# IN2-ViAUn/Exploration-of-Potential

Measured on AMD Instinct MI355X. Metric: training images/sec, YOLOX-l 24p 640x640 bf16, higher is better.
Workload: dtype bf16; 1 GPU; YOLOX-l-24p (CSPDarknet53+PAFPN+24p head) train step, 640x640, batch 20/GPU, 10 GTs/img, SimOTA + 24-circle GIoU loss, SGD nesterov; global_batch=20, parallelism=dp1, hip_graph=forward and backward as two lanes of captured segments, loss, update

## Files before the change

### exploration-of-potential_amd/csrc/elementwise.hip

```cpp
#include <stdio.h>
#include <stdlib.h>
#include "common.h"

namespace {

constexpr int MAX_BLOCKS = 2048;

__device__ __forceinline__ void load8(const bf16* p, float (&v)[8]) {
    bf16x8 t = *reinterpret_cast<const bf16x8*>(p);
#pragma unroll
    for (int i = 0; i < 8; ++i) v[i] = (float)t[i];
}
__device__ __forceinline__ void store8(bf16* p, const float (&v)[8]) {
    bf16x8 t;
#pragma unroll
    for (int i = 0; i < 8; ++i) t[i] = (bf16)v[i];
    *reinterpret_cast<bf16x8*>(p) = t;
}

struct RowMap {
    int tpr, rpb;
    __device__ RowMap(int C, int nt = 256) { tpr = C >> 3; rpb = tpr >= nt ? 1 : nt / tpr; }
};

template <int ACT, bool RES>
__global__ __launch_bounds__(256) void bn_act_fwd_kernel(const bf16* z, long ld_z, const long long* stats, int reps,
                                                         const float* gamma, const float* beta, float* rmean,
                                                         float* rvar, long* nbt, long* nbt2, float* save, bf16* y, long ld_y,
                                                         const bf16* res_, long ld_res, long M, int C, float eps,
                                                         float momentum) {
    constexpr int act = ACT;
    const bf16* res = RES ? res_ : nullptr;
    extern __shared__ float lds[];
    const int CP = C + (C >> 3);
    float* sc = lds;
    float* sh = lds + CP;
    auto pad = [](int c) { return c + (c >> 3); };
    for (int c = threadIdx.x; c < C; c += 256) {
        long long i1 = 0, i2 = 0;
        const float gmm = gamma[c], bta = beta[c];
        for (int rb = 0; rb < reps; rb += 8) {
            long long a[8], b[8];
#pragma unroll
            for (int r = 0; r < 8; ++r) {
                const int rr = rb + r < reps ? rb + r : rb;
                a[r] = stats[(long)rr * 2 * C + c];
                b[r] = stats[(long)rr * 2 * C + C + c];
            }
#pragma unroll
            for (int r = 0; r < 8; ++r) {
                i1 += rb + r < reps ? a[r] : 0ll;
                i2 += rb + r < reps ? b[r] : 0ll;
            }
        }
        const float mean = from_fix(i1) / (float)M;
        float var = from_fix(i2) / (float)M - mean * mean;
        var = var < 0.f ? 0.f : var;
        const float invstd = rsqrtf(var + eps);
        const float s_ = gmm * invstd;
        sc[pad(c)] = s_;
        sh[pad(c)] = bta - mean * s_;
        if (blockIdx.x == 0) {
            save[c] = mean;
            save[C + c] = invstd;
            if (rmean) {
                const float unb = M > 1 ? var * (float)M / (float)(M - 1) : var;
                rmean[c] = (1.f - momentum) * rmean[c] + momentum * mean;
                rvar[c] = (1.f - momentum) * rvar[c] + momentum * unb;
            }
        }
    }
    if (blockIdx.x == 0 && threadIdx.x == 0) {
        if (nbt) *nbt += 1;
        if (nbt2) *nbt2 += 1;
    }
    __syncthreads();
    const int cgs = C >> 3;
    const long total = M * cgs;
    const long stride = (long)gridDim.x * 256;
    constexpr int U = 4;
    const bool fixed_group = stride % cgs == 0;
    const int g_fixed = (int)(((long)blockIdx.x * 256 + threadIdx.x) % cgs);
    float rsc[8], rsh[8];
#pragma unroll
    for (int j = 0; j < 8; ++j) { rsc[j] = sc[g_fixed * 9 + j]; rsh[j] = sh[g_fixed * 9 + j]; }
    const long m_fixed = ((long)blockIdx.x * 256 + threadIdx.x) / cgs, m_step = stride / cgs;
    int it = 0;
    for (long i = (long)blockIdx.x * 256 + threadIdx.x; i < total; i += U * stride, ++it) {
        long mm[U];
        int gg[U];
        bf16x8 v[U], r[U];
#pragma unroll
        for (int k = 0; k < U; ++k) {
            const long ik = i + k * stride;
            const bool ok = ik < total;
            if (fixed_group) {
                mm[k] = ok ? m_fixed + (long)(it * U + k) * m_step : -1;
                gg[k] = g_fixed;
            } else {
                mm[k] = ok ? ik / cgs : -1;
                gg[k] = ok ? (int)(ik - mm[k] * cgs) : 0;
            }
            if (ok) {
                v[k] = *reinterpret_cast<const bf16x8*>(z + mm[k] * ld_z + gg[k] * 8);
                if constexpr (RES) r[k] = *reinterpret_cast<const bf16x8*>(res + mm[k] * ld_res + gg[k] * 8);
            }
        }
#pragma unroll
        for (int k = 0; k < U; ++k) {
            if (mm[k] < 0) break;
            bf16x8 o;
#pragma unroll
            for (int j = 0; j < 8; ++j) {
                const float a_ = fixed_group ? rsc[j] : sc[gg[k] * 9 + j];
                const float b_ = fixed_group ? rsh[j] : sh[gg[k] * 9 + j];
                const float u = fmaf((float)v[k][j], a_, b_);
                if constexpr (RES) o[j] = (bf16)(act_fwd(u, act) + (float)r[k][j]);
                else o[j] = (bf16)act_fwd(u, act);
            }
            *reinterpret_cast<bf16x8*>(y + mm[k] * ld_y + gg[k] * 8) = o;
        }
    }
}


template <int UNROLL, int NT, int ACT>
__device__ __forceinline__ void bn_bwd_reduce_body(const bf16* dy, long ld_dy, const bf16* z, long ld_z,
                                                   const float* save, const float* gamma,
                                                   const float* beta, long long* dgamma, long long* dbeta,
                                                   long M, int C, int reps, const int bid, const int nblk) {
    constexpr int act = ACT;
    __shared__ float red[NT][8 + 1];
    const RowMap rm(C, NT);
    const int tid = threadIdx.x;
    for (int cg0 = 0; cg0 < (C >> 3); cg0 += NT) {
        const int cg = cg0 + tid % rm.tpr;
        const int slot = rm.tpr >= NT ? 0 : tid / rm.tpr;
        const bool active = slot < rm.rpb && cg < (C >> 3);
        float sg[8] = {0, 0, 0, 0, 0, 0, 0, 0}, sb[8] = {0, 0, 0, 0, 0, 0, 0, 0};
        if (active) {
            const long step = (long)nblk * rm.rpb;
            const long m_first = (long)bid * rm.rpb + slot;
            bf16x8 vdy[UNROLL], vz[UNROLL];
#pragma unroll
            for (int k = 0; k < UNROLL; ++k) {
                const long mm = m_first + k * step < M ? m_first + k * step : (m_first < M ? m_first : 0);
                vdy[k] = *reinterpret_cast<const bf16x8*>(dy + mm * ld_dy + cg * 8);
                vz[k] = *reinterpret_cast<const bf16x8*>(z + mm * ld_z + cg * 8);
            }
            __builtin_amdgcn_sched_barrier(0);
            float sc[8], sh[8], iv[8], mi[8];
#pragma unroll
            for (int j = 0; j < 8; ++j) {
                const int c = cg * 8 + j;
                const float mean = save[c], inv = save[C + c];
                sc[j] = gamma[c] * inv; sh[j] = beta[c] - mean * sc[j]; iv[j] = inv; mi[j] = mean * inv;
            }
            for (long m = m_first; m < M; m += UNROLL * step) {
#pragma unroll
                for (int k = 0; k < UNROLL; ++k) {
                    if (m + k * step >= M) break;
#pragma unroll
                    for (int j = 0; j < 8; ++j) {
                        const float zz = (float)vz[k][j];
                        const float du = (float)vdy[k][j] * act_grad(fmaf(zz, sc[j], sh[j]), act);
                        sb[j] += du;
                        sg[j] = fmaf(du, fmaf(zz, iv[j], -mi[j]), sg[j]);
                    }
                }
                if (m + UNROLL * step < M) {
#pragma unroll
                    for (int k = 0; k < UNROLL; ++k) {
                        const long mn = m + (UNROLL + k) * step;
                        const long mm = mn < M ? mn : m;
                        vdy[k] = *reinterpret_cast<const bf16x8*>(dy + mm * ld_dy + cg * 8);
                        vz[k] = *reinterpret_cast<const bf16x8*>(z + mm * ld_z + cg * 8);
                    }
                }
            }
        }
        const int ngrp = min(min(rm.tpr, NT), (C >> 3) - cg0);
#pragma unroll
        for (int half = 0; half < 2; ++half) {
#pragma unroll
            for (int j = 0; j < 8; ++j) red[tid][j] = half ? sb[j] : sg[j];
            __syncthreads();
            for (int t = tid; t < ngrp * 8; t += NT) {
                const int g = t >> 3, v = t & 7;
                float a = 0.f;
                for (int sl = 0; sl < rm.rpb; ++sl) a += red[sl * rm.tpr + g][v];
                long long* dst = (half ? dbeta : dgamma) + (long)(bid % reps) * 2 * C + (cg0 + g) * 8 + v;
                atomicAdd((unsigned long long*)dst, (unsigned long long)to_fix_g(a));
            }
            __syncthreads();
        }
    }
}

template <int UNROLL, int NT, int ACT>
__global__ __launch_bounds__(NT) void bn_act_bwd_reduce_kernel(const bf16* dy, long ld_dy, const bf16* z, long ld_z,
                                                               const float* save, const float* gamma,
                                                               const float* beta, long long* dgamma, long long* dbeta,
                                                               long M, int C, int reps) {
    bn_bwd_reduce_body<UNROLL, NT, ACT>(dy, ld_dy, z, ld_z, save, gamma, beta, dgamma, dbeta, M, C, reps, (int)blockIdx.x, (int)gridDim.x);
}

template <int UNROLL, int ACT, bool ACC, bool COH>
__device__ __forceinline__ void bn_bwd_apply_body(const bf16* dy, long ld_dy, const bf16* z, long ld_z,
                                                  const float* save, const float* gamma, const float* beta,
                                                  const long long* dgamma, const long long* dbeta, float* ggrad,
                                                  float* bgrad, bf16* dz, long ld_dz, long M, int C, int reps, const int bid, const int nblk) {
    constexpr int act = ACT;
    const RowMap rm(C);
    const int tid = threadIdx.x;
    const float invM = 1.f / (float)M;
    extern __shared__ float folded[];
    for (int i = tid; i < 2 * C; i += 256) {
        const long long* src = i < C ? dgamma + i : dbeta + (i - C);
        long long acc = 0;
        bool bad = false;
        for (int rb = 0; rb < reps; rb += 8) {
            long long a[8];
#pragma unroll
            for (int r = 0; r < 8; ++r) {
                const long long* q = src + (long)(rb + r < reps ? rb + r : rb) * 2 * C;
                a[r] = COH ? __hip_atomic_load(q, __ATOMIC_RELAXED, __HIP_MEMORY_SCOPE_AGENT) : *q;
            }
#pragma unroll
            for (int r = 0; r < 8; ++r) {
                acc += rb + r < reps ? a[r] : 0ll;
                bad = bad || fixg_bad(a[r]);
            }
        }
        folded[i] = bad ? __builtin_nanf("") : from_fix_g(acc);
    }
    __syncthreads();
    for (int cg = tid % rm.tpr; cg < (C >> 3); cg += 256) {
        const int slot = rm.tpr >= 256 ? 0 : tid / rm.tpr;
        if (slot >= rm.rpb) break;
        float sc[8], sh[8], k1[8], k2[8], k3[8];
        float cm[8], ci[8], cg_[8], cb[8], csg[8], csb[8];
        {
            const f32x4* pm = reinterpret_cast<const f32x4*>(save + cg * 8);
            const f32x4* pi = reinterpret_cast<const f32x4*>(save + C + cg * 8);
            const f32x4* pg = reinterpret_cast<const f32x4*>(gamma + cg * 8);
            const f32x4* pb = reinterpret_cast<const f32x4*>(beta + cg * 8);
            const f32x4 m0 = pm[0], m1 = pm[1], i0 = pi[0], i1 = pi[1], g0 = pg[0], g1 = pg[1], b0 = pb[0], b1 = pb[1];
            const f32x4 s0 = *reinterpret_cast<const f32x4*>(folded + cg * 8), s1 = *reinterpret_cast<const f32x4*>(folded + cg * 8 + 4);
            const f32x4 t0 = *reinterpret_cast<const f32x4*>(folded + C + cg * 8), t1 = *reinterpret_cast<const f32x4*>(folded + C + cg * 8 + 4);
#pragma unroll
            for (int j = 0; j < 4; ++j) {
                cm[j] = m0[j]; cm[4 + j] = m1[j]; ci[j] = i0[j]; ci[4 + j] = i1[j]; cg_[j] = g0[j]; cg_[4 + j] = g1[j]; cb[j] = b0[j]; cb[4 + j] = b1[j];
                csg[j] = s0[j]; csg[4 + j] = s1[j]; csb[j] = t0[j]; csb[4 + j] = t1[j];
            }
        }
#pragma unroll
        for (int j = 0; j < 8; ++j) {
            const float mean = cm[j], inv = ci[j], g = cg_[j];
            const float sg_ = csg[j], sb_ = csb[j];
            sc[j] = g * inv; sh[j] = cb[j] - mean * sc[j];
            k1[j] = g * inv;
            k3[j] = k1[j] * inv * (sg_ * invM);
            k2[j] = k1[j] * (sb_ * invM) - k3[j] * mean;
        }
        if (bid == 0 && slot == 0 && ggrad) {
            f32x4* pgg = reinterpret_cast<f32x4*>(ggrad + cg * 8);
            f32x4* pbg = reinterpret_cast<f32x4*>(bgrad + cg * 8);
            f32x4 a0 = pgg[0], a1 = pgg[1], c0 = pbg[0], c1 = pbg[1];
#pragma unroll
            for (int j = 0; j < 4; ++j) {
                a0[j] += csg[j]; a1[j] += csg[4 + j];
                c0[j] += csb[j]; c1[j] += csb[4 + j];
            }
            pgg[0] = a0; pgg[1] = a1; pbg[0] = c0; pbg[1] = c1;
        }
        const long step = (long)nblk * rm.rpb;
        for (long m = (long)bid * rm.rpb + slot; m < M; m += UNROLL * step) {
            bf16x8 vdy[UNROLL], vz[UNROLL];
#pragma unroll
            for (int k = 0; k < UNROLL; ++k) {
                const long mm = m + k * step;
                if (mm < M) {
                    vdy[k] = __builtin_nontemporal_load(reinterpret_cast<const bf16x8*>(dy + mm * ld_dy + cg * 8));
                    vz[k] = __builtin_nontemporal_load(reinterpret_cast<const bf16x8*>(z + mm * ld_z + cg * 8));
                }
            }
#pragma unroll
            for (int k = 0; k < UNROLL; ++k) {
                const long mm = m + k * step;
                if (mm >= M) break;
                bf16x8 o;
#pragma unroll
                for (int j = 0; j < 8; ++j) {
                    const float zz = (float)vz[k][j];
                    const float du = (float)vdy[k][j] * act_grad(fmaf(zz, sc[j], sh[j]), act);
                    o[j] = (bf16)fmaf(-k3[j], zz, fmaf(k1[j], du, -k2[j]));
                }
                if (ACC) {
                    const bf16x8 old = *reinterpret_cast<const bf16x8*>(dz + mm * ld_dz + cg * 8);
#pragma unroll
                    for (int j = 0; j < 8; ++j) o[j] = (bf16)((float)old[j] + (float)o[j]);
                }
                *reinterpret_cast<bf16x8*>(dz + mm * ld_dz + cg * 8) = o;
            }
        }
    }
}

template <int UNROLL, int ACT, bool ACC = false>
__global__ __launch_bounds__(256) void bn_act_bwd_apply_kernel(const bf16* dy, long ld_dy, const bf16* z, long ld_z,
                                                               const float* save, const float* gamma, const float* beta,
                                                               const long long* dgamma, const long long* dbeta, float* ggrad,
                                                               float* bgrad, bf16* dz, long ld_dz, long M, int C, int reps) {
    bn_bwd_apply_body<UNROLL, ACT, ACC, false>(dy, ld_dy, z, ld_z, save, gamma, beta, dgamma, dbeta, ggrad, bgrad, dz, ld_dz, M, C, reps,
                                               (int)blockIdx.x, (int)gridDim.x);
}

__device__ unsigned g_bn_barrier_timeouts;

template <int ACT>
__global__ __launch_bounds__(256) void bn_act_bwd_fused_kernel(const bf16* dy, long ld_dy, const bf16* z, long ld_z,
                                                               const float* save, const float* gamma, const float* beta,
                                                               long long* dgamma, long long* dbeta, float* ggrad, float* bgrad,
                                                               bf16* dz, long ld_dz, long M, int C, int reps, unsigned* bar) {
    const int bid = (int)blockIdx.x, nblk = (int)gridDim.x;
    bn_bwd_reduce_body<4, 256, ACT>(dy, ld_dy, z, ld_z, save, gamma, beta, dgamma, dbeta, M, C, reps, bid, nblk);
    __syncthreads();
    if (threadIdx.x == 0) {
        __threadfence();
        __hip_atomic_fetch_add(bar, 1u, __ATOMIC_RELEASE, __HIP_MEMORY_SCOPE_AGENT);
        int tries = 0;
        while (__hip_atomic_load(bar, __ATOMIC_ACQUIRE, __HIP_MEMORY_SCOPE_AGENT) < (unsigned)nblk) {
            __builtin_amdgcn_s_sleep(2);
            if (++tries > (1 << 16)) { atomicAdd(&g_bn_barrier_timeouts, 1u); break; }
        }
    }
    __syncthreads();
    bn_bwd_apply_body<4, ACT, false, true>(dy, ld_dy, z, ld_z, save, gamma, beta, dgamma, dbeta, ggrad, bgrad, dz, ld_dz, M, C, reps, bid, nblk);
}

int flat_grid(long M, int C, int per_thread) {
    long blocks = (M * (C >> 3) + 256L * per_thread - 1) / (256L * per_thread);
    return (int)(blocks < 1 ? 1 : (blocks > MAX_BLOCKS ? MAX_BLOCKS : blocks));
}
int rows_grid(long M, int C, int rows_per_thread, int max_blocks, int nt = 256) {
    int tpr = C >> 3;
    int rpb = tpr >= nt ? 1 : nt / tpr;
    long blocks = (M + (long)rpb * rows_per_thread - 1) / ((long)rpb * rows_per_thread);
    return (int)(blocks < 1 ? 1 : (blocks > max_blocks ? max_blocks : blocks));
}

__global__ __launch_bounds__(256) void stem_pack_kernel(const float* img, bf16* rows, int B, int IH, int IW, int ld) {
    constexpr int TP = 32;
    __shared__ __attribute__((aligned(16))) bf16 tile[TP][120];
    const int FH = IH >> 1, FW = IW >> 1;
    const long npix = (long)B * FH * FW;
    const int chunks = ld >> 3;
    for (long p0 = (long)blockIdx.x * TP; p0 < npix; p0 += (long)gridDim.x * TP) {
        for (int it = threadIdx.x; it < 9 * TP; it += 256) {
            const int tap = it / TP, lp = it - tap * TP;
            const long pix = p0 + lp;
            float v[12] = {0.f, 0.f, 0.f, 0.f, 0.f, 0.f, 0.f, 0.f, 0.f, 0.f, 0.f, 0.f};
            if (pix < npix) {
                const int n = (int)(pix / ((long)FH * FW));
                const int rem = (int)(pix - (long)n * FH * FW);
                const int oy = rem / FW, ox = rem - oy * FW;
                const int fy = oy + tap / 3 - 1, fx = ox + tap % 3 - 1;
                if (fy >= 0 && fy < FH && fx >= 0 && fx < FW) {
#pragma unroll
                    for (int ch = 0; ch < 3; ++ch)
#pragma unroll
                        for (int yp = 0; yp < 2; ++yp) {
                            const float2 t = *reinterpret_cast<const float2*>(img + (((long)n * 3 + ch) * IH + 2 * fy + yp) * IW + 2 * fx);
                            v[(0 * 2 + yp) * 3 + ch] = t.x;
                            v[(1 * 2 + yp) * 3 + ch] = t.y;
                        }
                }
            }
#pragma unroll
            for (int j = 0; j < 12; ++j) tile[lp][tap * 12 + j] = (bf16)v[j];
        }
        if (threadIdx.x < TP) {
#pragma unroll
            for (int j = 108; j < 120; ++j) tile[threadIdx.x][j] = (bf16)0.f;
        }
        __syncthreads();
        for (int it = threadIdx.x; it < TP * chunks; it += 256) {
            const int lp = it / chunks, c = it - lp * chunks;
            const long pix = p0 + lp;
            if (pix >= npix) continue;
            bf16x8 o = {0, 0, 0, 0, 0, 0, 0, 0};
            if (c * 8 < 120) o = *reinterpret_cast<const bf16x8*>(&tile[lp][c * 8]);
            *reinterpret_cast<bf16x8*>(rows + pix * ld + c * 8) = o;
        }
        __syncthreads();
    }
}

__global__ __launch_bounds__(256) void focus_pack_kernel(const float* img, bf16* out, int B, int IH, int IW) {
    const int FH = IH >> 1, FW = IW >> 1;
    const long npix = (long)B * FH * FW;
    for (long pix = (long)blockIdx.x * 256 + threadIdx.x; pix < npix; pix += (long)gridDim.x * 256) {
        const int n = (int)(pix / ((long)FH * FW));
        const int rem = (int)(pix - (long)n * FH * FW);
        const int fy = rem / FW, fx = rem - fy * FW;
        float v[12];
#pragma unroll
        for (int ch = 0; ch < 3; ++ch)
#pragma unroll
            for (int yp = 0; yp < 2; ++yp) {
                const float2 t = *reinterpret_cast<const float2*>(img + (((long)n * 3 + ch) * IH + 2 * fy + yp) * IW + 2 * fx);
                v[(0 * 2 + yp) * 3 + ch] = t.x;
                v[(1 * 2 + yp) * 3 + ch] = t.y;
            }
        bf16x8 lo, hi = {0, 0, 0, 0, 0, 0, 0, 0};
#pragma unroll
        for (int j = 0; j < 8; ++j) lo[j] = (bf16)v[j];
#pragma unroll
        for (int j = 8; j < 12; ++j) hi[j - 8] = (bf16)v[j];
        *reinterpret_cast<bf16x8*>(out + pix * 16) = lo;
        *reinterpret_cast<bf16x8*>(out + pix * 16 + 8) = hi;
    }
}

__global__ __launch_bounds__(256) void spp_fwd_kernel(const bf16* x, long ld_x, bf16* y5, bf16* y9, bf16* y13, long ld_y,
                                                      uint8_t* idx, int B, int H, int W, int C) {
    const int cgs = C >> 3;
    const long total = (long)B * H * W * cgs;
    const long plane = (long)B * H * W * C;
    for (long i = (long)blockIdx.x * 256 + threadIdx.x; i < total; i += (long)gridDim.x * 256) {
        const int cg = (int)(i % cgs);
        const long pix = i / cgs;
        const int n = (int)(pix / (H * W));
        const int rem = (int)(pix - (long)n * H * W);
        const int py = rem / W, px = rem - py * W;
        float m5[8], m9[8], m13[8];
        uint8_t i5[8], i9[8], i13[8];
#pragma unroll
        for (int j = 0; j < 8; ++j) { m5[j] = m9[j] = m13[j] = -INFINITY; i5[j] = i9[j] = i13[j] = 0x88; }
        for (int dy = -6; dy <= 6; ++dy) {
            const int yy = py + dy;
            if (yy < 0 || yy >= H) continue;
            for (int dx = -6; dx <= 6; ++dx) {
                const int xx = px + dx;
                if (xx < 0 || xx >= W) continue;
                float v[8];
                load8(x + ((long)(n * H + yy) * W + xx) * ld_x + cg * 8, v);
                const uint8_t code = (uint8_t)(((dy + 8) << 4) | (dx + 8));
                const bool in9 = dy >= -4 && dy <= 4 && dx >= -4 && dx <= 4;
                const bool in5 = dy >= -2 && dy <= 2 && dx >= -2 && dx <= 2;
#pragma unroll
                for (int j = 0; j < 8; ++j) {
                    if (v[j] > m13[j] || v[j] != v[j]) { m13[j] = v[j]; i13[j] = code; }
                    if (in9 && (v[j] > m9[j] || v[j] != v[j])) { m9[j] = v[j]; i9[j] = code; }
                    if (in5 && (v[j] > m5[j] || v[j] != v[j])) { m5[j] = v[j]; i5[j] = code; }
                }
            }
        }
        store8(y5 + pix * ld_y + cg * 8, m5);
        store8(y9 + pix * ld_y + cg * 8, m9);
        store8(y13 + pix * ld_y + cg * 8, m13);
        uint8_t* ip = idx + pix * C + cg * 8;
#pragma unroll
        for (int j = 0; j < 8; ++j) { ip[j] = i5[j]; ip[plane + j] = i9[j]; ip[2 * plane + j] = i13[j]; }
    }
}

__global__ __launch_bounds__(256) void spp_row_kernel(const bf16* x, long ld_x, bf16* h, uint8_t* hx, int B, int H, int W, int C) {
    const int cgs = C >> 3;
    const long total = (long)B * H * W * cgs;
    const long plane = (long)B * H * W * C;
    for (long i = (long)blockIdx.x * 256 + threadIdx.x; i < total; i += (long)gridDim.x * 256) {
        const int cg = (int)(i % cgs);
        const long pix = i / cgs;
        const int px = (int)(pix % W);
        float m5[8], m9[8], m13[8];
        uint8_t i5[8], i9[8], i13[8];
#pragma unroll
        for (int j = 0; j < 8; ++j) { m5[j] = m9[j] = m13[j] = -INFINITY; i5[j] = i9[j] = i13[j] = 8; }
#pragma unroll
        for (int dx = -6; dx <= 6; ++dx) {
            const int xx = px + dx;
            if (xx < 0 || xx >= W) continue;
            float v[8];
            load8(x + (pix + dx) * ld_x + cg * 8, v);
            const uint8_t code = (uint8_t)(dx + 8);
            const bool in9 = dx >= -4 && dx <= 4, in5 = dx >= -2 && dx <= 2;
#pragma unroll
            for (int j = 0; j < 8; ++j) {
                if (v[j] > m13[j] || v[j] != v[j]) { m13[j] = v[j]; i13[j] = code; }
                if (in9 && (v[j] > m9[j] || v[j] != v[j])) { m9[j] = v[j]; i9[j] = code; }
// ... 465 lines not shown
        }
        const long* d = desc + (long)sg * 8;
        const int Cout = (int)d[3], T = (int)d[4], Cin = (int)d[5];
        const int tci = (Cin + 63) >> 6, tco = (Cout + 63) >> 6;
        long r = tl - tprefix[sg];
        const int ci0 = (int)(r % tci) * 64; r /= tci;
        const int co0 = (int)(r % tco) * 64;
        const int t = (int)(r / tco);
        const int c = threadIdx.x & 63, r4 = threadIdx.x >> 6;
        const long src0 = d[0];
        if ((Cin & 3) == 0 && (src0 & 3) == 0) {
#pragma unroll
            for (int k = 0; k < 4; ++k) {
                const int idx = threadIdx.x + 256 * k;
                const int row = idx >> 4, c4 = (idx & 15) * 4;
                const int co = co0 + row, ci = ci0 + c4;
                f32x4 v = {0.f, 0.f, 0.f, 0.f};
                if (co < Cout && ci < Cin) v = *reinterpret_cast<const f32x4*>(flat + src0 + ((long)co * T + t) * Cin + ci);
                tile[row][c4] = v[0]; tile[row][c4 + 1] = v[1]; tile[row][c4 + 2] = v[2]; tile[row][c4 + 3] = v[3];
            }
        } else {
#pragma unroll
            for (int k = 0; k < 16; ++k) {
                const int co = co0 + r4 + 4 * k, ci = ci0 + c;
                tile[r4 + 4 * k][c] = (co < Cout && ci < Cin) ? flat[src0 + ((long)co * T + t) * Cin + ci] : 0.f;
            }
        }
        __syncthreads();
        if (d[2] >= 0) {
            const int cop = (int)d[7];
            if ((cop & 7) == 0 && (d[2] & 7) == 0) {
#pragma unroll
                for (int k = 0; k < 2; ++k) {
                    const int idx = threadIdx.x + 256 * k;
                    const int cl = idx >> 3, j = idx & 7;
                    const int ci = ci0 + cl, co = co0 + 8 * j;
                    if (ci < Cin && co < cop) {
                        bf16x8 o;
#pragma unroll
                        for (int e = 0; e < 8; ++e) o[e] = (bf16)tile[8 * j + e][cl];
                        *reinterpret_cast<bf16x8*>(wd + d[2] + ((long)ci * T + t) * cop + co) = o;
                    }
                }
            } else {
#pragma unroll
                for (int k = 0; k < 16; ++k) {
                    const int ci = ci0 + r4 + 4 * k, co = co0 + c;
                    if (ci < Cin && co < Cout) wd[d[2] + ((long)ci * T + t) * cop + co] = (bf16)tile[c][r4 + 4 * k];
                }
            }
        }
        __syncthreads();
    }
}

__device__ __forceinline__ float ema_step(float e, float pnew, float d, float omd) {
    return __fadd_rn(__fmul_rn(e, d), __fmul_rn(omd, pnew));
}

constexpr int WF_NONE = -2147483647 - 1;
struct DecayArgs { float decay; const uint8_t* grp; };
template <bool DECAY, typename... X>
__global__ __launch_bounds__(256) void sgd_kernel(float* p, const float* g, float* buf, long n, float lr, float mom,
                                                  float gscale, const int* first_flag, const float* hp, float* ema,
                                                  long base, const int* wf_delta, bf16* wf, X... x) {
    float decay = 0.f;
    const uint8_t* decay_grp = nullptr;
    if constexpr (DECAY) {
        const DecayArgs t{x...};
        decay = t.decay;
        decay_grp = t.grp;
    }
    const int first = *first_flag;
    float d = 0.f, omd = 0.f;
    if (hp) {
        lr = hp[0]; mom = hp[1]; gscale = hp[2]; d = hp[3]; omd = hp[4];
        if (DECAY) decay = hp[5];
    }
    for (long i = ((long)blockIdx.x * 256 + threadIdx.x) * 4; i < n; i += (long)gridDim.x * 1024) {
        if (i + 3 < n) {
            f32x4 gv = *reinterpret_cast<const f32x4*>(g + i);
            f32x4 pv = *reinterpret_cast<const f32x4*>(p + i);
            f32x4 bv = first ? (f32x4){0.f, 0.f, 0.f, 0.f} : *reinterpret_cast<const f32x4*>(buf + i);
            const int wd = wf_delta ? wf_delta[(base + i) >> 6] : WF_NONE;
            const bool dec = DECAY && decay_grp[(base + i) >> 6] != 0;
#pragma unroll
            for (int j = 0; j < 4; ++j) {
                float gg = gv[j] * gscale;
                if (DECAY) gg = dec ? gg + decay * pv[j] : gg;
                bv[j] = first ? gg : mom * bv[j] + gg;
                pv[j] -= lr * (gg + mom * bv[j]);
            }
            *reinterpret_cast<f32x4*>(buf + i) = bv;
            *reinterpret_cast<f32x4*>(p + i) = pv;
            if (wd != WF_NONE) {
                bf16x4 o;
#pragma unroll
                for (int j = 0; j < 4; ++j) o[j] = (bf16)pv[j];
                *reinterpret_cast<bf16x4*>(wf + (base + i + wd)) = o;
            }
            if (ema) {
                f32x4 ev = *reinterpret_cast<const f32x4*>(ema + i);
#pragma unroll
                for (int j = 0; j < 4; ++j) ev[j] = ema_step(ev[j], pv[j], d, omd);
                *reinterpret_cast<f32x4*>(ema + i) = ev;
            }
        } else {
            for (long k = i; k < n; ++k) {
                float gg = g[k] * gscale;
                if (DECAY) gg = decay_grp[(base + k) >> 6] != 0 ? gg + decay * p[k] : gg;
                const float b = first ? gg : mom * buf[k] + gg;
                buf[k] = b;
                p[k] -= lr * (gg + mom * b);
                if (ema) ema[k] = ema_step(ema[k], p[k], d, omd);
                const int wd = wf_delta ? wf_delta[(base + k) >> 6] : WF_NONE;
                if (wd != WF_NONE) wf[base + k + wd] = (bf16)p[k];
            }
        }
    }
}

__global__ __launch_bounds__(256) void ema_kernel(float* ema, const float* src, long n, float d, float omd, const float* hp) {
    if (hp) { d = hp[3]; omd = hp[4]; }
    for (long i = (long)blockIdx.x * 256 + threadIdx.x; i < n; i += (long)gridDim.x * 256) ema[i] = ema_step(ema[i], src[i], d, omd);
}

__global__ void set_hparams_kernel(float* hp, float lr, float mom, float gscale, float d, float omd) {
    hp[0] = lr; hp[1] = mom; hp[2] = gscale; hp[3] = d; hp[4] = omd;
}
__global__ void set_hparams_decay_kernel(float* hp, float lr, float mom, float gscale, float d, float omd, float decay) {
    hp[0] = lr; hp[1] = mom; hp[2] = gscale; hp[3] = d; hp[4] = omd; hp[5] = decay;
}
__global__ void clear_flag_kernel(int* f) { *f = 0; }

int cap_grid(long work_items) {
    long b = (work_items + 255) / 256;
    return (int)(b < 1 ? 1 : (b > MAX_BLOCKS ? MAX_BLOCKS : b));
}

}

#define S_ (hipStream_t) stream

extern "C" int ep24_bn_act_fwd(const void* z, int64_t ld_z, const int64_t* stats, int reps, const float* gamma,
                               const float* beta, float* running_mean, float* running_var, int64_t* num_batches,
                               int64_t* num_batches2, float* save, void* y, int64_t ld_y, const void* residual, int64_t ld_res,
                               int64_t M, int C, float eps, float momentum, int act, void* stream) {
    EP24_REQUIRE(act >= 0 && act <= 3, EP24_E_ARG, "bn_act_fwd: act=%d is none of 0 identity, 1 SiLU, 2 ReLU, 3 LeakyReLU(0.1)", act);
    EP24_REQUIRE(z && stats && gamma && beta && save && y, EP24_E_ARG, "bn_act_fwd: null pointer");
    EP24_REQUIRE(C % 8 == 0 && ld_z % 8 == 0 && ld_y % 8 == 0 && (!residual || ld_res % 8 == 0), EP24_E_ARG,
                 "bn_act_fwd: C=%d / strides must be multiples of 8", C);
    EP24_REQUIRE(M > 0 && reps > 0, EP24_E_ARG, "bn_act_fwd: empty");
    const int fw_per = (C >= 1024 || (C <= 128 && M * C >= (12L << 20))) ? 8 : 4;
    auto kfn = residual ? (act == 1 ? bn_act_fwd_kernel<1, true> : act == 2 ? bn_act_fwd_kernel<2, true> : act == 3 ? bn_act_fwd_kernel<3, true> : bn_act_fwd_kernel<0, true>)
                        : (act == 1 ? bn_act_fwd_kernel<1, false> : act == 2 ? bn_act_fwd_kernel<2, false> : act == 3 ? bn_act_fwd_kernel<3, false> : bn_act_fwd_kernel<0, false>);
    hipLaunchKernelGGL(kfn, dim3(flat_grid(M, C, fw_per)), dim3(256), 2 * (C + C / 8) * sizeof(float), S_, (const bf16*)z, ld_z, (const long long*)stats, reps, gamma,
                       beta, running_mean, running_var, (long*)num_batches, (long*)num_batches2, save, (bf16*)y, ld_y, (const bf16*)residual,
                       ld_res, M, C, eps, momentum);
    EP24_LAUNCH_CHECK("ep24_bn_act_fwd");
    return EP24_OK;
}

extern "C" int ep24_bn_act_bwd_reduce(const void* dy, int64_t ld_dy, const void* z, int64_t ld_z, const float* save,
                                      const float* gamma, const float* beta, int64_t* dgamma, int64_t* dbeta, int64_t M, int C,
                                      int act, int reps, void* stream) {
    EP24_REQUIRE(act >= 0 && act <= 3, EP24_E_ARG, "bn_act_bwd_reduce: act=%d is none of 0 identity, 1 SiLU, 2 ReLU, 3 LeakyReLU(0.1)", act);
    EP24_REQUIRE(dy && z && save && gamma && beta && dgamma && dbeta && reps > 0, EP24_E_ARG, "bn_act_bwd_reduce: null pointer / reps");
    EP24_REQUIRE(C % 8 == 0 && ld_dy % 8 == 0 && ld_z % 8 == 0, EP24_E_ARG, "bn_act_bwd_reduce: alignment");
    int red_cap = 512;
    int red_rows = 4;
    auto kfn = act == 1 ? bn_act_bwd_reduce_kernel<4, 256, 1> : act == 2 ? bn_act_bwd_reduce_kernel<4, 256, 2> : act == 3 ? bn_act_bwd_reduce_kernel<4, 256, 3> : bn_act_bwd_reduce_kernel<4, 256, 0>;
    hipLaunchKernelGGL(kfn, dim3(rows_grid(M, C, red_rows, red_cap, 256)), dim3(256), 0, S_, (const bf16*)dy, ld_dy, (const bf16*)z, ld_z,
                       save, gamma, beta, (long long*)dgamma, (long long*)dbeta, M, C, reps);
    EP24_LAUNCH_CHECK("ep24_bn_act_bwd_reduce");
    return EP24_OK;
}

extern "C" int ep24_bn_act_bwd_apply(const void* dy, int64_t ld_dy, const void* z, int64_t ld_z, const float* save,
                                     const float* gamma, const float* beta, const int64_t* dgamma, const int64_t* dbeta,
                                     float* gamma_grad, float* beta_grad, void* dz, int64_t ld_dz, int64_t M, int C, int act,
                                     int reps, void* stream) {
    EP24_REQUIRE(act >= 0 && act <= 3, EP24_E_ARG, "bn_act_bwd_apply: act=%d is none of 0 identity, 1 SiLU, 2 ReLU, 3 LeakyReLU(0.1)", act);
    EP24_REQUIRE(dy && z && save && gamma && beta && dgamma && dbeta && dz && reps > 0, EP24_E_ARG, "bn_act_bwd_apply: null pointer / reps");
    EP24_REQUIRE(C % 8 == 0 && ld_dy % 8 == 0 && ld_z % 8 == 0 && ld_dz % 8 == 0, EP24_E_ARG, "bn_act_bwd_apply: alignment");
    EP24_REQUIRE((((uintptr_t)save | (uintptr_t)gamma | (uintptr_t)beta) & 15) == 0, EP24_E_ARG,
                 "bn_act_bwd_apply: save / gamma / beta must be 16-byte aligned (they are read as vectors)");
    EP24_REQUIRE((((uintptr_t)gamma_grad | (uintptr_t)beta_grad) & 15) == 0, EP24_E_ARG, "bn_act_bwd_apply: gamma_grad / beta_grad must be 16-byte aligned");
    const int ap_rows = M * C <= (16L << 20) ? 8 : 16, ap_cap = 2048;
    auto kfn = act == 1 ? bn_act_bwd_apply_kernel<4, 1> : act == 2 ? bn_act_bwd_apply_kernel<4, 2> : act == 3 ? bn_act_bwd_apply_kernel<4, 3> : bn_act_bwd_apply_kernel<4, 0>;
    hipLaunchKernelGGL(kfn, dim3(rows_grid(M, C, ap_rows, ap_cap)), dim3(256), 2 * (size_t)C * sizeof(float), S_, (const bf16*)dy, ld_dy,
                       (const bf16*)z, ld_z, save, gamma, beta, (const long long*)dgamma, (const long long*)dbeta, gamma_grad, beta_grad,
                       (bf16*)dz, ld_dz, M, C, reps);
    EP24_LAUNCH_CHECK("ep24_bn_act_bwd_apply");
    return EP24_OK;
}

extern "C" int ep24_bn_act_bwd_fused(const void* dy, int64_t ld_dy, const void* z, int64_t ld_z, const float* save, const float* gamma,
                                     const float* beta, int64_t* dgamma, int64_t* dbeta, float* gamma_grad, float* beta_grad, void* dz,
                                     int64_t ld_dz, int64_t M, int C, int act, int reps, int32_t* barrier, void* stream) {
    EP24_REQUIRE(act >= 0 && act <= 3, EP24_E_ARG, "bn_act_bwd_fused: act=%d is none of 0 identity, 1 SiLU, 2 ReLU, 3 LeakyReLU(0.1)", act);
    EP24_REQUIRE(dy && z && save && gamma && beta && dgamma && dbeta && dz && barrier && reps > 0, EP24_E_ARG, "bn_act_bwd_fused: null pointer / reps");
    EP24_REQUIRE(C % 8 == 0 && C <= 2048 && ld_dy % 8 == 0 && ld_z % 8 == 0 && ld_dz % 8 == 0, EP24_E_ARG, "bn_act_bwd_fused: alignment / C <= 2048");
    EP24_REQUIRE((((uintptr_t)save | (uintptr_t)gamma | (uintptr_t)beta | (uintptr_t)gamma_grad | (uintptr_t)beta_grad) & 15) == 0, EP24_E_ARG,
                 "bn_act_bwd_fused: save / gamma / beta and their gradients must be 16-byte aligned (they are read as vectors)");
    int grid = rows_grid(M, C, 4, 256, 256);
    auto kfn = act == 1 ? bn_act_bwd_fused_kernel<1> : act == 2 ? bn_act_bwd_fused_kernel<2> : act == 3 ? bn_act_bwd_fused_kernel<3> : bn_act_bwd_fused_kernel<0>;
    hipLaunchKernelGGL(kfn, dim3(grid), dim3(256), 2 * (size_t)C * sizeof(float), S_, (const bf16*)dy, ld_dy, (const bf16*)z, ld_z, save, gamma, beta,
                       (long long*)dgamma, (long long*)dbeta, gamma_grad, beta_grad, (bf16*)dz, ld_dz, M, C, reps, (unsigned*)barrier);
    EP24_LAUNCH_CHECK("ep24_bn_act_bwd_fused");
    return EP24_OK;
}

namespace ep24_igemm {
int bn_barrier_timeouts() {
    unsigned v = 0;
    if (hipMemcpyFromSymbol(&v, HIP_SYMBOL(g_bn_barrier_timeouts), sizeof(v)) != hipSuccess) return -1;
    return (int)v;
}
}

extern "C" int ep24_bn_act_bwd_apply_acc(const void* dy, int64_t ld_dy, const void* z, int64_t ld_z, const float* save,
                                         const float* gamma, const float* beta, const int64_t* dgamma, const int64_t* dbeta,
                                         float* gamma_grad, float* beta_grad, void* dz, int64_t ld_dz, int64_t M, int C, int act,
                                         int reps, void* stream) {
    EP24_REQUIRE(act >= 0 && act <= 3, EP24_E_ARG, "bn_act_bwd_apply_acc: act=%d is none of 0 identity, 1 SiLU, 2 ReLU, 3 LeakyReLU(0.1)", act);
    EP24_REQUIRE(dy && z && save && gamma && beta && dgamma && dbeta && dz && reps > 0, EP24_E_ARG, "bn_act_bwd_apply_acc: null pointer / reps");
    EP24_REQUIRE(C % 8 == 0 && ld_dy % 8 == 0 && ld_z % 8 == 0 && ld_dz % 8 == 0, EP24_E_ARG, "bn_act_bwd_apply_acc: alignment");
    EP24_REQUIRE((((uintptr_t)save | (uintptr_t)gamma | (uintptr_t)beta) & 15) == 0, EP24_E_ARG,
                 "bn_act_bwd_apply_acc: save / gamma / beta must be 16-byte aligned (they are read as vectors)");
    EP24_REQUIRE((((uintptr_t)gamma_grad | (uintptr_t)beta_grad) & 15) == 0, EP24_E_ARG, "bn_act_bwd_apply_acc: gamma_grad / beta_grad must be 16-byte aligned");
    auto kfn = act == 1 ? bn_act_bwd_apply_kernel<4, 1, true> : act == 2 ? bn_act_bwd_apply_kernel<4, 2, true> : act == 3 ? bn_act_bwd_apply_kernel<4, 3, true> : bn_act_bwd_apply_kernel<4, 0, true>;
    hipLaunchKernelGGL(kfn, dim3(rows_grid(M, C, 16, 2048)), dim3(256), 2 * (size_t)C * sizeof(float), S_, (const bf16*)dy, ld_dy, (const bf16*)z, ld_z, save, gamma, beta,
                       (const long long*)dgamma, (const long long*)dbeta, gamma_grad, beta_grad, (bf16*)dz, ld_dz, M, C, reps);
    EP24_LAUNCH_CHECK("ep24_bn_act_bwd_apply_acc");
    return EP24_OK;
}

extern "C" int ep24_stem_pack(const float* images, void* rows, int64_t ld, int B, int H, int W, void* stream) {
    EP24_REQUIRE(images && rows && H % 2 == 0 && W % 2 == 0 && B > 0 && ld >= 108 && ld % 8 == 0, EP24_E_ARG, "stem_pack: bad arguments");
    long sp_blocks = ((long)B * (H / 2) * (W / 2) + 31) / 32;
    hipLaunchKernelGGL(stem_pack_kernel, dim3((unsigned)(sp_blocks > 16384 ? 16384 : sp_blocks)), dim3(256), 0, S_, images,
                       (bf16*)rows, B, H, W, (int)ld);
    EP24_LAUNCH_CHECK("ep24_stem_pack");
    return EP24_OK;
}

extern "C" int ep24_focus_pack(const float* images, void* f16, int B, int H, int W, void* stream) {
    EP24_REQUIRE(images && f16 && H % 2 == 0 && W % 2 == 0 && B > 0 && (reinterpret_cast<unsigned long long>(images) & 7) == 0, EP24_E_ARG,
                 "focus_pack: bad arguments");
    const long blocks = ((long)B * (H / 2) * (W / 2) + 255) / 256;
    hipLaunchKernelGGL(focus_pack_kernel, dim3((unsigned)(blocks > 65536 ? 65536 : blocks)), dim3(256), 0, S_, images, (bf16*)f16, B, H, W);
    EP24_LAUNCH_CHECK("ep24_focus_pack");
    return EP24_OK;
}

extern "C" int ep24_spp_fwd(const void* x, int64_t ld_x, void* y5, void* y9, void* y13, int64_t ld_y, uint8_t* idx, int B,
                            int H, int W, int C, void* scratch, void* stream) {
    EP24_REQUIRE(x && y5 && y9 && y13 && idx && C % 8 == 0 && ld_x % 8 == 0 && ld_y % 8 == 0, EP24_E_ARG, "spp_fwd: bad arguments");
    if (scratch) {
        const long n = (long)B * H * W * C;
        bf16* h = (bf16*)scratch;
        uint8_t* hx = (uint8_t*)scratch + 6 * n;
        hipLaunchKernelGGL(spp_row_kernel, dim3(cap_grid(n / 8)), dim3(256), 0, S_, (const bf16*)x, ld_x, h, hx, B, H, W, C);
        hipLaunchKernelGGL(spp_col_kernel, dim3(cap_grid(n / 8)), dim3(256), 0, S_, (const bf16*)h, (const uint8_t*)hx, (bf16*)y5,
                           (bf16*)y9, (bf16*)y13, ld_y, idx, B, H, W, C);
        EP24_LAUNCH_CHECK("ep24_spp_fwd");
        return EP24_OK;
    }
    hipLaunchKernelGGL(spp_fwd_kernel, dim3(cap_grid((long)B * H * W * (C / 8))), dim3(256), 0, S_, (const bf16*)x, ld_x,
                       (bf16*)y5, (bf16*)y9, (bf16*)y13, ld_y, idx, B, H, W, C);
    EP24_LAUNCH_CHECK("ep24_spp_fwd");
    return EP24_OK;
}

extern "C" int ep24_spp_bwd(const void* dy5, const void* dy9, const void* dy13, int64_t ld_dy, const uint8_t* idx, void* dx,
                            int64_t ld_dx, int accumulate, int B, int H, int W, int C, void* stream) {
    EP24_REQUIRE(dy5 && dy9 && dy13 && idx && dx && C % 8 == 0 && ld_dy % 8 == 0 && ld_dx % 8 == 0, EP24_E_ARG, "spp_bwd: bad arguments");
    const size_t lds = (size_t)H * W * 112;
    if (lds <= 64 * 1024 && H * W <= 1024)
        hipLaunchKernelGGL(spp_bwd_lds_kernel, dim3(C / 8, B), dim3(256), lds, S_, (const bf16*)dy5, (const bf16*)dy9, (const bf16*)dy13,
                           ld_dy, idx, (bf16*)dx, ld_dx, accumulate, B, H, W, C);
    else
        hipLaunchKernelGGL(spp_bwd_kernel, dim3(cap_grid((long)B * H * W * (C / 8))), dim3(256), 0, S_, (const bf16*)dy5,
                           (const bf16*)dy9, (const bf16*)dy13, ld_dy, idx, (bf16*)dx, ld_dx, accumulate, B, H, W, C);
    EP24_LAUNCH_CHECK("ep24_spp_bwd");
    return EP24_OK;
}

extern "C" int ep24_upsample2_fwd(const void* x, int64_t ld_x, void* y, int64_t ld_y, int B, int H, int W, int C, void* stream) {
    EP24_REQUIRE(x && y && C % 8 == 0 && ld_x % 8 == 0 && ld_y % 8 == 0, EP24_E_ARG, "upsample2_fwd: bad arguments");
    hipLaunchKernelGGL(upsample2_fwd_kernel, dim3(cap_grid((long)B * 4 * H * W * (C / 8))), dim3(256), 0, S_, (const bf16*)x,
                       ld_x, (bf16*)y, ld_y, B, H, W, C);
    EP24_LAUNCH_CHECK("ep24_upsample2_fwd");
    return EP24_OK;
}

extern "C" int ep24_upsample2_bwd(const void* dy, int64_t ld_dy, void* dx, int64_t ld_dx, int accumulate, int B, int H, int W,
                                  int C, void* stream) {
    EP24_REQUIRE(dy && dx && C % 8 == 0 && ld_dy % 8 == 0 && ld_dx % 8 == 0, EP24_E_ARG, "upsample2_bwd: bad arguments");
    hipLaunchKernelGGL(upsample2_bwd_kernel, dim3(cap_grid((long)B * H * W * (C / 8))), dim3(256), 0, S_, (const bf16*)dy, ld_dy,
                       (bf16*)dx, ld_dx, accumulate, B, H, W, C);
    EP24_LAUNCH_CHECK("ep24_upsample2_bwd");
    return EP24_OK;
}

extern "C" int ep24_rows_copy(const void* src, int64_t ld_src, void* dst, int64_t ld_dst, int accumulate, int64_t M, int C,
                              void* stream) {
    EP24_REQUIRE(src && dst && C % 8 == 0 && ld_src % 8 == 0 && ld_dst % 8 == 0, EP24_E_ARG, "rows_copy: bad arguments");
    hipLaunchKernelGGL(rows_copy_kernel, dim3(cap_grid(M * (C / 8))), dim3(256), 0, S_, (const bf16*)src, ld_src, (bf16*)dst,
// ... 213 lines not shown
```

Measured before the change: 1023 images/s.

## Software-pipeline BN forward/backward loops with incremental cursors and occupancy hints

The BN+activation forward kernel now uses a compile-time FIXED template flag and incremental offset cursors in place of per-element division. Its loop is rotated so each slot's next load is issued right after the previous slot is finished. The backward reduce and apply kernels get the same rotated prefetch structure with sched_barriers and a separate tail loop, and waves-per-EU hints are added. The aim is to hide global memory latency and cut integer address arithmetic in these bandwidth-bound kernels, at the cost of more template instantiations and register pressure.

```diff
diff --git a/exploration-of-potential_amd/csrc/elementwise.hip b/exploration-of-potential_amd/csrc/elementwise.hip
--- a/exploration-of-potential_amd/csrc/elementwise.hip
+++ b/exploration-of-potential_amd/csrc/elementwise.hip
@@ -16,6 +16,11 @@
 #pragma unroll
     for (int i = 0; i < 8; ++i) t[i] = (bf16)v[i];
     *reinterpret_cast<bf16x8*>(p) = t;
+}
+
+__device__ __forceinline__ long pinned_row(long m) {
+    asm volatile("" : "+v"(m));
+    return m;
 }
 
 struct RowMap {
@@ -23,7 +28,7 @@
     __device__ RowMap(int C, int nt = 256) { tpr = C >> 3; rpb = tpr >= nt ? 1 : nt / tpr; }
 };
 
-template <int ACT, bool RES>
+template <int ACT, bool RES, bool FIXED>
 __global__ __launch_bounds__(256) void bn_act_fwd_kernel(const bf16* z, long ld_z, const long long* stats, int reps,
                                                          const float* gamma, const float* beta, float* rmean,
                                                          float* rvar, long* nbt, long* nbt2, float* save, bf16* y, long ld_y,
@@ -75,54 +80,85 @@
         if (nbt2) *nbt2 += 1;
     }
     __syncthreads();
-    const int cgs = C >> 3;
+    const unsigned cgs = (unsigned)C >> 3;
     const long total = M * cgs;
-    const long stride = (long)gridDim.x * 256;
+    const unsigned nthr = gridDim.x * 256u;
+    const unsigned t0 = blockIdx.x * 256u + threadIdx.x;
+    if ((long)t0 >= total) return;
     constexpr int U = 4;
-    const bool fixed_group = stride % cgs == 0;
-    const int g_fixed = (int)(((long)blockIdx.x * 256 + threadIdx.x) % cgs);
+    const unsigned qs = nthr / cgs, rs = FIXED ? 0u : nthr - qs * cgs;
+    const unsigned row0 = t0 / cgs, g0 = t0 - row0 * cgs;
     float rsc[8], rsh[8];
-#pragma unroll
-    for (int j = 0; j < 8; ++j) { rsc[j] = sc[g_fixed * 9 + j]; rsh[j] = sh[g_fixed * 9 + j]; }
-    const long m_fixed = ((long)blockIdx.x * 256 + threadIdx.x) / cgs, m_step = stride / cgs;
-    int it = 0;
-    for (long i = (long)blockIdx.x * 256 + threadIdx.x; i < total; i += U * stride, ++it) {
-        long mm[U];
-        int gg[U];
-        bf16x8 v[U], r[U];
+    if constexpr (FIXED) {
+#pragma unroll
+        for (int j = 0; j < 8; ++j) { rsc[j] = sc[g0 * 9 + j]; rsh[j] = sh[g0 * 9 + j]; }
+    }
+    struct Cursor {
+        long i, off;
+        unsigned g;
+    };
+    auto advance = [&](Cursor& c, long step, long carry) {
+        c.i += nthr;
+        c.off += step;
+        if constexpr (!FIXED) {
+            c.g += rs;
+            const bool wrap = c.g >= cgs;
+            c.g -= wrap ? cgs : 0u;
+            c.off += wrap ? carry : 0l;
+        }
+    };
+    const long step_z = (long)qs * ld_z + rs * 8, carry_z = ld_z - C;
+    const long step_y = (long)qs * ld_y + rs * 8, carry_y = ld_y - C;
+    const long step_r = RES ? (long)qs * ld_res + rs * 8 : 0, carry_r = RES ? ld_res - C : 0;
+    const long first_z = (long)row0 * ld_z + g0 * 8, first_r = RES ? (long)row0 * ld_res + g0 * 8 : 0;
+    Cursor lz{(long)t0, first_z, g0}, lr{(long)t0, first_r, g0};
+    Cursor st{(long)t0, (long)row0 * ld_y + g0 * 8, g0};
+    bf16x8 v[U], r[U];
+    auto request = [&](int k) {
+        const bool ok = lz.i < total;
+        v[k] = *reinterpret_cast<const bf16x8*>(z + (ok ? lz.off : first_z));
+        advance(lz, step_z, carry_z);
+        if constexpr (RES) {
+            r[k] = *reinterpret_cast<const bf16x8*>(res + (ok ? lr.off : first_r));
+            advance(lr, step_r, carry_r);
+        }
+    };
+    auto finish = [&](int k) {
+        bf16x8 o;
+#pragma unroll
+        for (int j = 0; j < 8; ++j) {
+            const float a_ = FIXED ? rsc[j] : sc[st.g * 9 + j];
+            const float b_ = FIXED ? rsh[j] : sh[st.g * 9 + j];
+            const float u = fmaf((float)v[k][j], a_, b_);
+            if constexpr (RES) o[j] = (bf16)(act_fwd(u, act) + (float)r[k][j]);
+            else o[j] = (bf16)act_fwd(u, act);
+        }
+        *reinterpret_cast<bf16x8*>(y + st.off) = o;
+        advance(st, step_y, carry_y);
+    };
+#pragma unroll
+    for (int k = 0; k < U; ++k) {
+        request(k);
+        __builtin_amdgcn_sched_barrier(0);
+    }
+    while (st.i + (long)U * nthr < total) {
 #pragma unroll
         for (int k = 0; k < U; ++k) {
-            const long ik = i + k * stride;
-            const bool ok = ik < total;
-            if (fixed_group) {
-                mm[k] = ok ? m_fixed + (long)(it * U + k) * m_step : -1;
-                gg[k] = g_fixed;
-            } else {
-                mm[k] = ok ? ik / cgs : -1;
-                gg[k] = ok ? (int)(ik - mm[k] * cgs) : 0;
-            }
-            if (ok) {
-                v[k] = *reinterpret_cast<const bf16x8*>(z + mm[k] * ld_z + gg[k] * 8);
-                if constexpr (RES) r[k] = *reinterpret_cast<const bf16x8*>(res + mm[k] * ld_res + gg[k] * 8);
-            }
-        }
-#pragma unroll
-        for (int k = 0; k < U; ++k) {
-            if (mm[k] < 0) break;
-            bf16x8 o;
-#pragma unroll
-            for (int j = 0; j < 8; ++j) {
-                const float a_ = fixed_group ? rsc[j] : sc[gg[k] * 9 + j];
-                const float b_ = fixed_group ? rsh[j] : sh[gg[k] * 9 + j];
-                const float u = fmaf((float)v[k][j], a_, b_);
-                if constexpr (RES) o[j] = (bf16)(act_fwd(u, act) + (float)r[k][j]);
-                else o[j] = (bf16)act_fwd(u, act);
-            }
-            *reinterpret_cast<bf16x8*>(y + mm[k] * ld_y + gg[k] * 8) = o;
-        }
-    }
-}
-
+            finish(k);
+            __builtin_amdgcn_sched_barrier(0);
+            request(k);
+            __builtin_amdgcn_sched_barrier(0);
+        }
+    }
+#pragma unroll
+    for (int k = 0; k < U; ++k) {
+        if (st.i >= total) break;
+        finish(k);
+    }
+}
+
+
+#define EP24_BN_WAVES __attribute__((amdgpu_waves_per_eu(4)))
 
 template <int UNROLL, int NT, int ACT>
 __device__ __forceinline__ void bn_bwd_reduce_body(const bf16* dy, long ld_dy, const bf16* z, long ld_z,
@@ -140,13 +176,14 @@
         float sg[8] = {0, 0, 0, 0, 0, 0, 0, 0}, sb[8] = {0, 0, 0, 0, 0, 0, 0, 0};
         if (active) {
             const long step = (long)nblk * rm.rpb;
-            const long m_first = (long)bid * rm.rpb + slot;
+            const long m_first = pinned_row((long)bid * rm.rpb + slot);
             bf16x8 vdy[UNROLL], vz[UNROLL];
 #pragma unroll
             for (int k = 0; k < UNROLL; ++k) {
                 const long mm = m_first + k * step < M ? m_first + k * step : (m_first < M ? m_first : 0);
                 vdy[k] = *reinterpret_cast<const bf16x8*>(dy + mm * ld_dy + cg * 8);
                 vz[k] = *reinterpret_cast<const bf16x8*>(z + mm * ld_z + cg * 8);
+                __builtin_amdgcn_sched_barrier(0);
             }
             __builtin_amdgcn_sched_barrier(0);
             float sc[8], sh[8], iv[8], mi[8];
@@ -156,27 +193,33 @@
                 const float mean = save[c], inv = save[C + c];
                 sc[j] = gamma[c] * inv; sh[j] = beta[c] - mean * sc[j]; iv[j] = inv; mi[j] = mean * inv;
             }
-            for (long m = m_first; m < M; m += UNROLL * step) {
+            auto add_row = [&](int k) {
+#pragma unroll
+                for (int j = 0; j < 8; ++j) {
+                    if (j == 4) __builtin_amdgcn_sched_barrier(0);
+                    const float zz = (float)vz[k][j];
+                    const float du = (float)vdy[k][j] * act_grad(fmaf(zz, sc[j], sh[j]), act);
+                    sb[j] += du;
+                    sg[j] = fmaf(du, fmaf(zz, iv[j], -mi[j]), sg[j]);
+                }
+            };
+            long m = m_first;
+            for (; m + UNROLL * step < M; m += UNROLL * step) {
 #pragma unroll
                 for (int k = 0; k < UNROLL; ++k) {
-                    if (m + k * step >= M) break;
-#pragma unroll
-                    for (int j = 0; j < 8; ++j) {
-                        const float zz = (float)vz[k][j];
-                        const float du = (float)vdy[k][j] * act_grad(fmaf(zz, sc[j], sh[j]), act);
-                        sb[j] += du;
-                        sg[j] = fmaf(du, fmaf(zz, iv[j], -mi[j]), sg[j]);
-                    }
+                    add_row(k);
+                    __builtin_amdgcn_sched_barrier(0);
+                    const long mn = m + (UNROLL + k) * step;
+                    const long mm = mn < M ? mn : m + UNROLL * step;
+                    vdy[k] = *reinterpret_cast<const bf16x8*>(dy + mm * ld_dy + cg * 8);
+                    vz[k] = *reinterpret_cast<const bf16x8*>(z + mm * ld_z + cg * 8);
+                    __builtin_amdgcn_sched_barrier(0);
                 }
-                if (m + UNROLL * step < M) {
-#pragma unroll
-                    for (int k = 0; k < UNROLL; ++k) {
-                        const long mn = m + (UNROLL + k) * step;
-                        const long mm = mn < M ? mn : m;
-                        vdy[k] = *reinterpret_cast<const bf16x8*>(dy + mm * ld_dy + cg * 8);
-                        vz[k] = *reinterpret_cast<const bf16x8*>(z + mm * ld_z + cg * 8);
-                    }
-                }
+            }
+#pragma unroll
+            for (int k = 0; k < UNROLL; ++k) {
+                if (m + k * step >= M) break;
+                add_row(k);
             }
         }
         const int ngrp = min(min(rm.tpr, NT), (C >> 3) - cg0);
@@ -198,7 +241,7 @@
 }
 
 template <int UNROLL, int NT, int ACT>
-__global__ __launch_bounds__(NT) void bn_act_bwd_reduce_kernel(const bf16* dy, long ld_dy, const bf16* z, long ld_z,
+__global__ __launch_bounds__(NT) EP24_BN_WAVES void bn_act_bwd_reduce_kernel(const bf16* dy, long ld_dy, const bf16* z, long ld_z,
                                                                const float* save, const float* gamma,
                                                                const float* beta, long long* dgamma, long long* dbeta,
                                                                long M, int C, int reps) {
@@ -275,40 +318,56 @@
             pgg[0] = a0; pgg[1] = a1; pbg[0] = c0; pbg[1] = c1;
         }
         const long step = (long)nblk * rm.rpb;
-        for (long m = (long)bid * rm.rpb + slot; m < M; m += UNROLL * step) {
-            bf16x8 vdy[UNROLL], vz[UNROLL];
+        long m = (long)bid * rm.rpb + slot;
+        if (m >= M) continue;
+        bf16x8 vdy[UNROLL], vz[UNROLL];
+#pragma unroll
+        for (int k = 0; k < UNROLL; ++k) {
+            const long mm = m + k * step < M ? m + k * step : m;
+            vdy[k] = __builtin_nontemporal_load(reinterpret_cast<const bf16x8*>(dy + mm * ld_dy + cg * 8));
+            vz[k] = __builtin_nontemporal_load(reinterpret_cast<const bf16x8*>(z + mm * ld_z + cg * 8));
+            __builtin_amdgcn_sched_barrier(0);
+        }
+        auto row = [&](int k, bool refill) {
+            bf16* pdz = dz + (m + k * step) * ld_dz + cg * 8;
+            bf16x8 old;
+            if (ACC) old = *reinterpret_cast<const bf16x8*>(pdz);
+            bf16x8 o;
+#pragma unroll
+            for (int j = 0; j < 8; ++j) {
+                const float zz = (float)vz[k][j];
+                const float du = (float)vdy[k][j] * act_grad(fmaf(zz, sc[j], sh[j]), act);
+                o[j] = (bf16)fmaf(-k3[j], zz, fmaf(k1[j], du, -k2[j]));
+            }
+            if (ACC) {
+#pragma unroll
+                for (int j = 0; j < 8; ++j) o[j] = (bf16)((float)old[j] + (float)o[j]);
+            }
+            *reinterpret_cast<bf16x8*>(pdz) = o;
+            if (refill) {
+                const long mn = m + (UNROLL + k) * step;
+                const long mm = mn < M ? mn : m + UNROLL * step;
+                vdy[k] = __builtin_nontemporal_load(reinterpret_cast<const bf16x8*>(dy + mm * ld_dy + cg * 8));
+                vz[k] = __builtin_nontemporal_load(reinterpret_cast<const bf16x8*>(z + mm * ld_z + cg * 8));
+            }
+        };
+        for (; m + UNROLL * step < M; m += UNROLL * step) {
 #pragma unroll
             for (int k = 0; k < UNROLL; ++k) {
-                const long mm = m + k * step;
-                if (mm < M) {
-                    vdy[k] = __builtin_nontemporal_load(reinterpret_cast<const bf16x8*>(dy + mm * ld_dy + cg * 8));
-                    vz[k] = __builtin_nontemporal_load(reinterpret_cast<const bf16x8*>(z + mm * ld_z + cg * 8));
-                }
-            }
-#pragma unroll
-            for (int k = 0; k < UNROLL; ++k) {
-                const long mm = m + k * step;
-                if (mm >= M) break;
-                bf16x8 o;
-#pragma unroll
-                for (int j = 0; j < 8; ++j) {
-                    const float zz = (float)vz[k][j];
-                    const float du = (float)vdy[k][j] * act_grad(fmaf(zz, sc[j], sh[j]), act);
-                    o[j] = (bf16)fmaf(-k3[j], zz, fmaf(k1[j], du, -k2[j]));
-                }
-                if (ACC) {
-                    const bf16x8 old = *reinterpret_cast<const bf16x8*>(dz + mm * ld_dz + cg * 8);
-#pragma unroll
-                    for (int j = 0; j < 8; ++j) o[j] = (bf16)((float)old[j] + (float)o[j]);
-                }
-                *reinterpret_cast<bf16x8*>(dz + mm * ld_dz + cg * 8) = o;
-            }
+                row(k, true);
+                __builtin_amdgcn_sched_barrier(0);
+            }
+        }
+#pragma unroll
+        for (int k = 0; k < UNROLL; ++k) {
+            if (m + k * step >= M) break;
+            row(k, false);
         }
     }
 }
 
 template <int UNROLL, int ACT, bool ACC = false>
-__global__ __launch_bounds__(256) void bn_act_bwd_apply_kernel(const bf16* dy, long ld_dy, const bf16* z, long ld_z,
+__global__ __launch_bounds__(256) __attribute__((amdgpu_waves_per_eu(ACC && ACT ? 3 : 4))) void bn_act_bwd_apply_kernel(const bf16* dy, long ld_dy, const bf16* z, long ld_z,
                                                                const float* save, const float* gamma, const float* beta,
                                                                const long long* dgamma, const long long* dbeta, float* ggrad,
                                                                float* bgrad, bf16* dz, long ld_dz, long M, int C, int reps) {
@@ -319,7 +378,7 @@
 __device__ unsigned g_bn_barrier_timeouts;
 
 template <int ACT>
-__global__ __launch_bounds__(256) void bn_act_bwd_fused_kernel(const bf16* dy, long ld_dy, const bf16* z, long ld_z,
+__global__ __launch_bounds__(256) EP24_BN_WAVES void bn_act_bwd_fused_kernel(const bf16* dy, long ld_dy, const bf16* z, long ld_z,
                                                                const float* save, const float* gamma, const float* beta,
                                                                long long* dgamma, long long* dbeta, float* ggrad, float* bgrad,
                                                                bf16* dz, long ld_dz, long M, int C, int reps, unsigned* bar) {
@@ -337,6 +396,12 @@
     }
     __syncthreads();
     bn_bwd_apply_body<4, ACT, false, true>(dy, ld_dy, z, ld_z, save, gamma, beta, dgamma, dbeta, ggrad, bgrad, dz, ld_dz, M, C, reps, bid, nblk);
+}
+
+template <bool FIXED>
+auto fwd_kernel(int act, bool residual) {
+    return residual ? (act == 1 ? bn_act_fwd_kernel<1, true, FIXED> : act == 2 ? bn_act_fwd_kernel<2, true, FIXED> : act == 3 ? bn_act_fwd_kernel<3, true, FIXED> : bn_act_fwd_kernel<0, true, FIXED>)
+                    : (act == 1 ? bn_act_fwd_kernel<1, false, FIXED> : act == 2 ? bn_act_fwd_kernel<2, false, FIXED> : act == 3 ? bn_act_fwd_kernel<3, false, FIXED> : bn_act_fwd_kernel<0, false, FIXED>);
 }
 
 int flat_grid(long M, int C, int per_thread) {
@@ -1108,9 +1173,10 @@
                  "bn_act_fwd: C=%d / strides must be multiples of 8", C);
     EP24_REQUIRE(M > 0 && reps > 0, EP24_E_ARG, "bn_act_fwd: empty");
     const int fw_per = (C >= 1024 || (C <= 128 && M * C >= (12L << 20))) ? 8 : 4;
-    auto kfn = residual ? (act == 1 ? bn_act_fwd_kernel<1, true> : act == 2 ? bn_act_fwd_kernel<2, true> : act == 3 ? bn_act_fwd_kernel<3, true> : bn_act_fwd_kernel<0, true>)
-                        : (act == 1 ? bn_act_fwd_kernel<1, false> : act == 2 ? bn_act_fwd_kernel<2, false> : act == 3 ? bn_act_fwd_kernel<3, false> : bn_act_fwd_kernel<0, false>);
-    hipLaunchKernelGGL(kfn, dim3(flat_grid(M, C, fw_per)), dim3(256), 2 * (C + C / 8) * sizeof(float), S_, (const bf16*)z, ld_z, (const long long*)stats, reps, gamma,
+    const int grid = flat_grid(M, C, fw_per);
+    const bool fixed = (grid * 256L) % (C >> 3) == 0;
+    auto kfn = fixed ? fwd_kernel<true>(act, residual != nullptr) : fwd_kernel<false>(act, residual != nullptr);
+    hipLaunchKernelGGL(kfn, dim3(grid), dim3(256), 2 * (C + C / 8) * sizeof(float), S_, (const bf16*)z, ld_z, (const long long*)stats, reps, gamma,
                        beta, running_mean, running_var, (long*)num_batches, (long*)num_batches2, save, (bf16*)y, ld_y, (const bf16*)residual,
                        ld_res, M, C, eps, momentum);
     EP24_LAUNCH_CHECK("ep24_bn_act_fwd");
```

Result: faster. 1036 images/s (median of 6 runs) (+1.3%).
